# fims9000/SYNT_ISIC

Measured on AMD Instinct MI355X. Metric: images/sec at 3x64x64 T=1000 (DDPM reverse-diffusion sampling), higher is better.
Workload: dtype f32

## Files before the change

synt_isic_amd/csrc/api.cpp:

```cpp
#include <cstring>

#include "common.h"

namespace sisic {

static thread_local char g_err[1024] = "";

void set_error(const char* fmt, ...) {
    va_list ap;
    va_start(ap, fmt);
    vsnprintf(g_err, sizeof(g_err), fmt, ap);
    va_end(ap);
}

static hipEvent_t take_event(sisic_ctx* ctx) {
    if (!ctx->event_pool.empty()) {
        hipEvent_t e = ctx->event_pool.back();
        ctx->event_pool.pop_back();
        return e;
    }
    hipEvent_t e = nullptr;
    if (hipEventCreate(&e) != hipSuccess) return nullptr;
    return e;
}
// ... 52 lines not shown
    *out = nullptr;
    int n = 0;
    SISIC_HIP(hipGetDeviceCount(&n));
    SISIC_REQUIRE(device_id >= 0 && device_id < n, "sisic_create: device %d of %d", device_id, n);
    SISIC_HIP(hipSetDevice(device_id));
    hipDeviceProp_t prop;
    SISIC_HIP(hipGetDeviceProperties(&prop, device_id));
    SISIC_REQUIRE(std::strncmp(prop.gcnArchName, "gfx950", 6) == 0,
                  "sisic_create: device %d is %s; this library is built for gfx950 (MI355X) only", device_id,
                  prop.gcnArchName);
    auto* ctx = new sisic_ctx();
    ctx->device = device_id;
    ctx->num_cus = prop.multiProcessorCount;
    *out = ctx;
    return SISIC_OK;
}

int sisic_destroy(sisic_ctx* ctx) {
    if (!ctx) return SISIC_OK;
    (void)profile_collect(ctx);
    for (auto e : ctx->event_pool) (void)hipEventDestroy(e);
    for (auto& kv : ctx->splitk)
        if (kv.second.p) (void)hipFree(kv.second.p);
    delete ctx;
    return SISIC_OK;
}

int64_t sisic_conv_packed_numel(int Cout, int Cin, int ksize) {
    if (Cout <= 0 || Cin <= 0 || (ksize != 1 && ksize != 3 && ksize != 7)) return -1;
    return conv_packed_floats(Cout, Cin, ksize);
}

int sisic_conv_pack_weights(sisic_ctx* ctx, const float* w, int Cout, int Cin, int ksize, float* packed, void* stream) {
    SISIC_REQUIRE(ctx && w && packed && Cout > 0 && Cin > 0, "conv_pack_weights: bad arguments");
    return launch_conv_pack(ctx, w, Cout, Cin, ksize, packed, static_cast<hipStream_t>(stream));
}

int64_t sisic_conv_s2_numel(int Cout, int Cin) {
    if (Cout <= 0 || Cin <= 0) return -1;
    return conv_s2_packed_floats(Cout, Cin);
}

int sisic_conv_s2_pack(sisic_ctx* ctx, const float* w, int Cout, int Cin, float* out, void* stream) {
    SISIC_REQUIRE(ctx && w && out && Cout > 0 && Cin > 0, "conv_s2_pack: bad arguments");
    return launch_conv_s2_pack(ctx, w, Cout, Cin, out, static_cast<hipStream_t>(stream));
}
// ... 119 lines not shown
```

synt_isic_amd/csrc/common.h:

```cpp
#pragma once

#include <hip/hip_runtime.h>

#include <atomic>
#include <cstdarg>
#include <cstdint>
#include <cstdio>
#include <string>
#include <map>
#include <mutex>
#include <vector>

#include "../../include/sisic.h"

namespace sisic {

void set_error(const char* fmt, ...);

#define SISIC_HIP(call)                                                                   \
    do {                                                                                  \
        hipError_t _e = (call);                                                           \
        if (_e != hipSuccess) {                                                           \
            ::sisic::set_error("%s failed: %s (%s:%d)", #call, hipGetErrorString(_e),     \
                               __FILE__, __LINE__);                                       \
// ... 20 lines not shown
struct ProfileSlot {
    double ms = 0, bytes = 0, flops = 0, flops_exec = 0;
    int64_t launches = 0;
};

struct PendingEvent {
    hipEvent_t start, stop;
    int kind;
    int kind2;
};

}

struct sisic_ctx {
    int device = 0;
    int num_cus = 0;
    bool profiling = false;
    sisic::ProfileSlot prof[sisic::PK_COUNT];
    std::vector<sisic::PendingEvent> pending;
    std::vector<hipEvent_t> event_pool;
    struct SplitK { float* p = nullptr; size_t floats = 0; };
    std::map<hipStream_t, SplitK> splitk;
    std::mutex splitk_mutex;
    std::atomic<uint64_t> scratch_generation{0};
};

namespace sisic {

struct ProfileScope {
    sisic_ctx* ctx;
    hipStream_t stream;
    PendingEvent ev{};
    bool active = false;
    ProfileScope(sisic_ctx* c, hipStream_t s, int kind, double bytes, double flops, double flops_exec = -1.0, int kind2 = -1);
    ~ProfileScope();
};

int profile_collect(sisic_ctx* ctx);

inline int ensure_dynamic_lds(sisic_ctx* ctx, const void* kern, int bytes, std::atomic<uint64_t>& done) {
    const uint64_t bit = uint64_t(1) << (ctx->device & 63);
    if (done.load(std::memory_order_acquire) & bit) return SISIC_OK;
    SISIC_HIP(hipFuncSetAttribute(kern, hipFuncAttributeMaxDynamicSharedMemorySize, bytes));
    done.fetch_or(bit, std::memory_order_release);
    return SISIC_OK;
}
// ... 100 lines not shown
```

synt_isic_amd/csrc/conv_winograd.hip:

```cpp
#include <type_traits>

#include "common.h"
#include "gn_merge.h"
#include "pack_device.h"

#ifndef WINO_TIMING
#define WINO_TIMING 0
#endif
#define WINO_STAMP_SLOTS 10
#if WINO_TIMING
#define WINO_STAMP(slot)                                                                                   \
    do {                                                                                                   \
        unsigned long long t_;                                                                             \
        asm volatile("s_memtime %0\n\ts_waitcnt lgkmcnt(0)" : "=s"(t_)::"memory");                         \
        if (tid == 0) reinterpret_cast<unsigned long long*>(p.stats)[(size_t)blockIdx.x * WINO_STAMP_SLOTS + (slot)] = t_; \
    } while (0)
#else
#define WINO_STAMP(slot) do { } while (0)
#endif
#ifndef WINO_ABLATE
#define WINO_ABLATE 0
#endif

namespace sisic {
// ... 12 lines not shown
    int cout_pad;
    const float* bias;
    int Cout;
    const float* gn_scale;
    const float* gn_shift;
    int gn_silu;
    const float* chan_bias;
    int chan_bias_stride;
    const float* residual;
    int relu;
    float* out;
    float* stats;
    float* part;
    int ksplit;
    int groups_x, groups_y, groups_b, n_co_tiles, nwg, nchunks;
    int stagger;
    const float* fin_gamma;
    const float* fin_beta;
    float* fin_scale;
    float* fin_shift;
    float* fin_mean_rstd;
    int fin_groups;
    float fin_eps;
};

constexpr int W_CIC = 8;
constexpr int W_TILES = 64;
constexpr int W_CO = 64;
constexpr int W_SLAB = W_CIC * 16 * 64;

typedef const __attribute__((address_space(1))) char* gcptr_t;
typedef const __attribute__((address_space(1))) float* gfptr_t;
typedef float v4f_t __attribute__((ext_vector_type(4)));
typedef float v2f_t __attribute__((ext_vector_type(2)));
typedef const __attribute__((address_space(1))) v4f_t* gf4ptr_t;
typedef const __attribute__((address_space(1))) v2f_t* gf2ptr_t;
typedef __attribute__((address_space(1))) float* gfwptr_t;
typedef __attribute__((address_space(1))) v2f_t* gf2wptr_t;
__device__ __forceinline__ gcptr_t uniform_ptr(const void* ptr) {
    const unsigned long long v = reinterpret_cast<unsigned long long>(ptr);
    const unsigned lo = __builtin_amdgcn_readfirstlane((unsigned)v);
    const unsigned hi = __builtin_amdgcn_readfirstlane((unsigned)(v >> 32));
    return (gcptr_t)(((unsigned long long)hi << 32) | lo);
}

__device__ __forceinline__ float wsilu(float v) { return v * __builtin_amdgcn_rcpf(1.0f + __expf(-v)); }
// ... 964 lines not shown
```

synt_isic_amd/csrc/conv_winograd_bf3.inc:

```
template <int PRO>
struct Bf3Geom {
    static constexpr int CO_T = 64, NW = 16, THREADS = 1024;
    static constexpr int TY = 8, TX = 8, TILES = 64;
    static constexpr int HH = 18, HWD = 18, HROW = 20, HPL = 10;
    static constexpr int HPI = HH * HWD;
    static constexpr int HB1 = 2 * HH * HROW;
    static constexpr int CPS = 2 * HB1;
    static constexpr int H_FLOATS = (W_CIC / 2) * CPS;
    static constexpr int TPC = THREADS / W_CIC;
    static constexpr int EPT = (HPI + TPC - 1) / TPC;
    static constexpr int RCO = 16, ROUNDS = CO_T / RCO;
    static constexpr int M_ROUND = 16 * RCO * TILES;
    static constexpr int EPI_FLOATS = 2 * M_ROUND;
    static constexpr int GN_MAX_CH = 2048;
    static constexpr int UA_WAVE = 768;
    static constexpr int UA_BUF = NW * UA_WAVE;
    static constexpr int UA_OFF = H_FLOATS + 2 * GN_MAX_CH;
    static constexpr int LOOP_FLOATS = UA_OFF + 2 * UA_BUF;
    static constexpr int EPI_OFF = H_FLOATS;
    static constexpr int HOFF_OFF = (LOOP_FLOATS > EPI_OFF + EPI_FLOATS ? LOOP_FLOATS : EPI_OFF + EPI_FLOATS);
    static constexpr int FIN_OFF = HOFF_OFF + 2 * THREADS;
    static constexpr size_t LDS_BYTES = sizeof(float) * (size_t)(FIN_OFF + 2 * CO_T);
    static_assert(LDS_BYTES <= 160 * 1024, "bf16x3 Winograd: LDS");
};
// ... 6 lines not shown
#endif
#ifndef BF3Q_VAR
#define BF3Q_VAR 0
#endif
#ifndef BF3_VAR
#define BF3_VAR 0
#endif
#define BF3_STAMPS 16
#if WINO_TIMING
#define BF3_STAMP(slot)                                                                                    \
    do {                                                                                                   \
        unsigned long long t_;                                                                             \
        asm volatile("s_memtime %0\n\ts_waitcnt lgkmcnt(0)" : "=s"(t_)::"memory");                         \
        if (lane == 0) reinterpret_cast<unsigned long long*>(p.stats)[((size_t)BF3_STAMP_ITEM * 16 + wave_u) * BF3_STAMPS + (slot)] = t_; \
    } while (0)
#else
#define BF3_STAMP(slot) do { } while (0)
#endif
typedef short bf3_bf16x8 __attribute__((ext_vector_type(8)));
typedef unsigned bf3_u4 __attribute__((ext_vector_type(4)));
typedef float bf3_f2 __attribute__((ext_vector_type(2)));
typedef unsigned bf3_u2 __attribute__((ext_vector_type(2)));

template <int PRO, bool UPS = false>
__global__ void __launch_bounds__(1024, 4) conv_winograd_bf3_kernel(const WinoParams p) {
    using G = Bf3Geom<PRO>;
    extern __shared__ __attribute__((aligned(16))) float smem[];
    float* const H_lds = smem;
    float* const GN_lds = smem + G::H_FLOATS;
    float* const M_base = smem + G::EPI_OFF;

    int L = blockIdx.x;
    int co_t, gx, gy, b0, oy0, ox0, co0;
    auto decode = [&](const int l) {
        const int nwg = p.nwg;
        const int xcd = l & 7, slot = l >> 3, q = nwg >> 3, r = nwg & 7;
        const int work = (xcd < r ? xcd * (q + 1) : r * (q + 1) + (xcd - r) * q) + slot;
        co_t = work % p.n_co_tiles;
        int grp = work / p.n_co_tiles;
        gx = grp % p.groups_x;
        grp /= p.groups_x;
        gy = grp % p.groups_y;
        b0 = grp / p.groups_y;
        oy0 = gy * 2 * G::TY; ox0 = gx * 2 * G::TX;
        co0 = co_t * G::CO_T;
    };
    decode(L);
    const int n = p.nchunks;
    const int per_img = p.n_co_tiles * p.groups_x * p.groups_y;
    const int img_step = ((p.nwg & 7) == 0 && (int)(gridDim.x >> 3) % per_img == 0) ? (int)(gridDim.x >> 3) / per_img : 0;

    const int tid = threadIdx.x;
    const int lane = tid & 63, wave = tid >> 6;
    const int half = lane >> 5, l31 = lane & 31;
    const int wave_u = __builtin_amdgcn_readfirstlane(wave);
    const int HWin = p.Hin * p.Win, Cin = p.c0 + p.c1;
    auto fresh_lane = [] {
        int l;
        asm volatile("v_mbcnt_lo_u32_b32 %0, -1, 0\n\tv_mbcnt_hi_u32_b32 %0, -1, %0" : "=v"(l));
        return l;
    };
    float* const UA_lds = smem + G::UA_OFF + wave_u * G::UA_WAVE;
    const unsigned ua_lds_addr = __builtin_amdgcn_readfirstlane((unsigned)(size_t)(__attribute__((address_space(3))) float*)UA_lds);

    __amdgpu_buffer_rsrc_t rs0, rs1;
    const __amdgpu_buffer_rsrc_t rsu = __builtin_amdgcn_make_buffer_rsrc(const_cast<float*>(p.uw), 0, -1, 0x00020000);

    const int sci = wave_u >> 1;
    const int sl = tid & 127;
    unsigned goff[G::EPT];
    int hoff[G::EPT];
    auto plan = [&](auto full_tag) {
        constexpr bool FULL = decltype(full_tag)::value;
// ... 7 lines not shown
            const int y = oy0 - 1 + yy, x = ox0 - 1 + xx;
            const bool v = in && y >= 0 && y < p.Hc && x >= 0 && x < p.Wc;
            const int slot = yy * G::HROW + (xx & 1) * G::HPL + (xx >> 1);
            goff[i] = v ? 4u * (unsigned)((y >> (UPS ? 1 : 0)) * p.Win + (x >> (UPS ? 1 : 0))) : 0u;
            if constexpr (FULL) {
                hoff[i] = 2 * (v ? slot : (G::HPL - 1) + G::HPL * (sl_i & 1));
                if (in && !v) {
                    float* z = H_lds + (sci >> 1) * G::CPS + 2 * slot + (sci & 1);
                    z[0] = 0.0f;
                    z[G::HB1] = 0.0f;
                }
            }
        }
        if constexpr (FULL) {
            static_assert(G::EPT == 3, "three store offsets in two dwords");
            *reinterpret_cast<bf3_u2*>(smem + G::HOFF_OFF + 2 * ((wave_u >> 1) * G::TPC + sl_i)) =
                bf3_u2{(unsigned)hoff[0] | ((unsigned)hoff[1] << 16), (unsigned)hoff[2]};
        }
    };
    auto set_sources = [&] {
        rs0 = __builtin_amdgcn_make_buffer_rsrc(const_cast<float*>(p.in0 + (size_t)b0 * p.c0 * HWin), 0, -1, 0x00020000);
        rs1 = __builtin_amdgcn_make_buffer_rsrc(const_cast<float*>(p.in1 ? p.in1 + (size_t)b0 * p.c1 * HWin : p.in0), 0, -1, 0x00020000);
    };
    set_sources();
    plan(std::false_type{});

    const int pos = wave_u, pi = pos >> 2, pj = pos & 3;
    const bool live = !(UPS && (pi == 2 || pj == 2));
    const int ra = (pi == 0) ? 0 : (pi == 2 ? 2 : 1), rb = (pi == 2) ? 1 : (pi == 3 ? 3 : 2);
    const int ca = (pj == 0) ? 0 : (pj == 2 ? 2 : 1), cb = (pj == 2) ? 1 : (pj == 3 ? 3 : 2);
    const float sr = (pi == 1) ? 1.0f : -1.0f, sc = (pj == 1) ? 1.0f : -1.0f;
    const int col_a = (ca & 1) * G::HPL + (ca >> 1), col_b = (cb & 1) * G::HPL + (cb >> 1);
    const float *p_ac, *p_ae, *p_bc, *p_be;
    unsigned u_lane;
    auto lane_addresses = [&] {
        const int ln = fresh_lane();
        const int hf = ln >> 5, t31 = ln & 31, ty = t31 >> 3, tx = t31 & 7;
        const int xf_lane = (2 * hf) * G::CPS + 2 * ((2 * ty) * G::HROW + tx);
        p_ac = H_lds + xf_lane + 2 * (ra * G::HROW + col_a);
        p_ae = H_lds + xf_lane + 2 * (ra * G::HROW + col_b);
        p_bc = H_lds + xf_lane + 2 * (rb * G::HROW + col_a);
        p_be = H_lds + xf_lane + 2 * (rb * G::HROW + col_b);
        u_lane = 16u * (unsigned)ln;
    };
    lane_addresses();

    const int n_co32 = p.cout_pad >> 5;
// ... 115 lines not shown
                acc[x][nb] = __builtin_amdgcn_mfma_f32_32x32x16_bf16(__builtin_bit_cast(bf3_bf16x8, ua[x]), __builtin_bit_cast(bf3_bf16x8, b_mh), acc[x][nb], 0, 0, 0);
                if constexpr ((BF3_VAR & 4096) == 0)
                    acc[x][nb] = __builtin_amdgcn_mfma_f32_32x32x16_bf16(__builtin_bit_cast(bf3_bf16x8, a_hl), __builtin_bit_cast(bf3_bf16x8, b_lh), acc[x][nb], 0, 0, 0);
                if constexpr ((BF3_VAR & 512) != 0) {
                    if constexpr (INIT) {
                        const f32x16 zero = {0.0f, 0.0f, 0.0f, 0.0f, 0.0f, 0.0f, 0.0f, 0.0f, 0.0f, 0.0f, 0.0f, 0.0f, 0.0f, 0.0f, 0.0f, 0.0f};
                        acc[x][1] = __builtin_amdgcn_mfma_f32_32x32x16_bf16(__builtin_bit_cast(bf3_bf16x8, ua[x]), __builtin_bit_cast(bf3_bf16x8, b_hm), zero, 0, 0, 0);
                    } else {
                        acc[x][1] = __builtin_amdgcn_mfma_f32_32x32x16_bf16(__builtin_bit_cast(bf3_bf16x8, ua[x]), __builtin_bit_cast(bf3_bf16x8, b_hm), acc[x][1], 0, 0, 0);
                    }
                    acc[x][1] = __builtin_amdgcn_mfma_f32_32x32x16_bf16(__builtin_bit_cast(bf3_bf16x8, ua[x]), __builtin_bit_cast(bf3_bf16x8, b_mh), acc[x][1], 0, 0, 0);
                    acc[x][1] = __builtin_amdgcn_mfma_f32_32x32x16_bf16(__builtin_bit_cast(bf3_bf16x8, a_hl), __builtin_bit_cast(bf3_bf16x8, b_lh), acc[x][1], 0, 0, 0);
                }
            }
            if constexpr ((BF3_VAR & 256) != 0) __builtin_amdgcn_s_setprio(0);
        }
        __builtin_amdgcn_sched_barrier(0);
    };

    const int cor = wave_u;
    float gn_pre0 = 0.0f, gn_pre1 = 0.0f;
    auto prefetch_gn = [&] {
        if constexpr (PRO != 0) {
            const int ci = b0 * Cin + min(wave_u * 64 + fresh_lane(), Cin - 1);
            gn_pre0 = p.gn_scale[ci];
            gn_pre1 = p.gn_shift[ci];
        }
    };
    auto pin_requests = [&] {
#pragma unroll
        for (int i = 0; i < G::EPT; ++i) asm volatile("" : "+v"(hs[0].v[i]));
#pragma unroll
        for (int i = 0; i < G::EPT; ++i) asm volatile("" : "+v"(hs[1].v[i]));
        if constexpr (PRO != 0) asm volatile("" : "+v"(gn_pre0), "+v"(gn_pre1));
    };
    load_halo(0, hs[0]);
    if (live) fetch_u(0, 0);
    if (n > 1) load_halo(1, hs[1]);
    prefetch_gn();
    pin_requests();
    bool first = true;
    bool new_tile = true;
  for (;;) {
#define BF3_STAMP_ITEM L
    BF3_STAMP(0);
    if constexpr (UPS) {
#pragma unroll
        for (int x = 0; x < 2; ++x)
#pragma unroll
            for (int nb = 0; nb < 2; ++nb)
#pragma unroll
                for (int r = 0; r < 16; ++r) acc[x][nb][r] = 0.0f;
    }
    if (new_tile) plan(std::true_type{});
    {
        const bf3_u2 h = *reinterpret_cast<const bf3_u2*>(smem + G::HOFF_OFF + 2 * (wave_u * 64 + fresh_lane()));
        hoff[0] = (int)(h.x & 0xffffu); hoff[1] = (int)(h.x >> 16); hoff[2] = (int)h.y;
    }
    lane_addresses();
    const float tile_cnt = (float)(min(2 * G::TY, p.Hc - oy0) * min(2 * G::TX, p.Wc - ox0));
    const float inv_cnt = 1.0f / tile_cnt;

    if constexpr (PRO != 0) {
        const int c0t = wave_u * 64 + fresh_lane();
        if (c0t < n * W_CIC) {
            const bool cv = c0t < Cin;
            *reinterpret_cast<bf3_f2*>(GN_lds + 2 * c0t) = bf3_f2{cv ? gn_pre0 : 0.0f, cv ? gn_pre1 : 0.0f};
        }
        for (int c = c0t + G::THREADS; c < n * W_CIC; c += G::THREADS) {
            const bool cv = c < Cin;
            const int ci = b0 * Cin + min(c, Cin - 1);
            const float gsc = p.gn_scale[ci], gsh = p.gn_shift[ci];
            *reinterpret_cast<bf3_f2*>(GN_lds + 2 * c) = bf3_f2{cv ? gsc : 0.0f, cv ? gsh : 0.0f};
        }
    }
    if (!first && live) fetch_u(0, 0);
    first = false;
    if constexpr (PRO != 0) __syncthreads();
    stage_halo(0, 0, hs[0]);
    if (n > 2) load_halo(2, hs[0]);
    __syncthreads();
    BF3_STAMP(1);
    {
        auto body = [&](const int c, auto par_tag, auto steady_tag, auto init_tag) {
            constexpr int PAR = decltype(par_tag)::value;
            constexpr bool STEADY = decltype(steady_tag)::value;
            if (c == 2 + PAR) BF3_STAMP(2 + 4 * PAR);
            if constexpr (BF3_PRIO != 0) __builtin_amdgcn_s_setprio(3);
            if (live) {
                if constexpr ((BF3_VAR & 1) == 0) {
                    read_u(BF3_ONE_UA ? 0 : PAR, std::integral_constant<int, STEADY ? 3 : 0>{}, c == 0 && n > 2);
                    if constexpr (BF3_ONE_UA != 0) {
                        if (STEADY || c + 1 < n) {
                            asm volatile("s_waitcnt lgkmcnt(0)" ::: "memory");
                            fetch_u(c + 1, 0);
                        }
                    }
                }
            }
            if (live) compute_half(PAR, std::integral_constant<int, 0>{}, init_tag);
            if (STEADY || c + 1 < n) {
                if constexpr ((BF3_VAR & 4) == 0) stage_halo(c + 1, PAR ^ 1, hs[PAR ^ 1]);
                if constexpr ((BF3_VAR & 1) == 0 && BF3_ONE_UA == 0)
                    if (live) fetch_u(c + 1, PAR ^ 1);
// ... 13 lines not shown
        c = 1;
        for (; c + 4 < n; c += 2) {
            body(c, std::integral_constant<int, 1>{}, std::true_type{}, std::false_type{});
            body(c + 1, std::integral_constant<int, 0>{}, std::true_type{}, std::false_type{});
        }
        if (c < n) body(c, std::integral_constant<int, 1>{}, std::false_type{}, std::false_type{});
        if (c + 1 < n) body(c + 1, std::integral_constant<int, 0>{}, std::false_type{}, std::false_type{});
        if (c + 2 < n) body(c + 2, std::integral_constant<int, 1>{}, std::false_type{}, std::false_type{});
        if (c + 3 < n) body(c + 3, std::integral_constant<int, 0>{}, std::false_type{}, std::false_type{});
    }

    BF3_STAMP(10);
    if constexpr ((BF3_VAR & 16) != 0) {
        float t = 0.0f;
#pragma unroll
        for (int x = 0; x < 2; ++x)
#pragma unroll
            for (int nb = 0; nb < 2; ++nb)
#pragma unroll
                for (int r = 0; r < 16; ++r) t += acc[x][nb][r];
        if (t == 123.456f) p.out[tid] = t;
        return;
    }
    float eadd_v = 0.0f;
    {
        const int ln = fresh_lane();
        const int coc = min(co0 + (ln & 3) * G::RCO + cor, p.Cout - 1);
        const float* src = ln < 4 ? (p.bias ? p.bias + coc : nullptr)
                                  : (ln < 8 && p.chan_bias ? p.chan_bias + (size_t)b0 * p.chan_bias_stride + coc : nullptr);
        if (src) eadd_v = *src;
    }
    const int HWo = p.Hc * p.Wc;
    const int et = fresh_lane(), e_half = et >> 5, e_l31 = et & 31;
    const int ety = et >> 3, etx = et & 7;
    const int eoy = oy0 + 2 * ety, eox = ox0 + 2 * etx;
    const bool even_w = (p.Wc & 1) == 0;
    const bool has_res = p.residual != nullptr;
    unsigned ld_off[2][2], st_off[2][2];
    bool pin[2][2];
#pragma unroll
    for (int i = 0; i < 2; ++i)
#pragma unroll
        for (int j = 0; j < 2; ++j) {
            pin[i][j] = eoy + i < p.Hc && eox + j < p.Wc;
            ld_off[i][j] = 4u * (unsigned)(min(eoy + i, p.Hc - 1) * p.Wc + min(eox + j, p.Wc - (even_w ? 2 - j : 1)));
            st_off[i][j] = pin[i][j] ? ld_off[i][j] : 0x80000000u;
        }
    const __amdgpu_buffer_rsrc_t rso = __builtin_amdgcn_make_buffer_rsrc(p.out + (size_t)b0 * p.Cout * HWo, 0, 4 * p.Cout * HWo, 0x00020000);
    const __amdgpu_buffer_rsrc_t rsr = __builtin_amdgcn_make_buffer_rsrc(
        const_cast<float*>(has_res ? p.residual + (size_t)b0 * p.Cout * HWo : p.out), 0, 4 * p.Cout * HWo, 0x00020000);

    bf3_f2 eres[G::ROUNDS][2];
#pragma unroll
    for (int q = 0; q < G::ROUNDS; ++q) {
        const int coc = min(co0 + q * G::RCO + cor, p.Cout - 1);
        const unsigned soff = 4u * (unsigned)(coc * HWo);
#pragma unroll
        for (int i = 0; i < 2; ++i) eres[q][i] = bf3_f2{0.0f, 0.0f};
        if (has_res) {
            if (even_w) {
#pragma unroll
                for (int i = 0; i < 2; ++i)
                    eres[q][i] = __builtin_bit_cast(bf3_f2, __builtin_amdgcn_raw_buffer_load_b64(rsr, ld_off[i][0], soff, 0));
            } else {
#pragma unroll
                for (int i = 0; i < 2; ++i) {
                    eres[q][i].x = __builtin_bit_cast(float, __builtin_amdgcn_raw_buffer_load_b32(rsr, ld_off[i][0], soff, 0));
                    eres[q][i].y = __builtin_bit_cast(float, __builtin_amdgcn_raw_buffer_load_b32(rsr, ld_off[i][1], soff, 0));
                }
            }
        }
    }
    float eadd[G::ROUNDS];
#pragma unroll
    for (int q = 0; q < G::ROUNDS; ++q)
        eadd[q] = (0.0f + __uint_as_float(__builtin_amdgcn_readlane(__float_as_uint(eadd_v), q))) +
                  __uint_as_float(__builtin_amdgcn_readlane(__float_as_uint(eadd_v), 4 + q));
    const int co0_c = co0, b0_c = b0, slot_c = gy * p.groups_x + gx;
    const int L_next = L + (int)gridDim.x;
    const bool more = L_next < p.nwg;
    if (more) {
        const int gx_c = gx, gy_c = gy;
        if (img_step) b0 += img_step;
        else decode(L_next);
        set_sources();
        new_tile = gx != gx_c || gy != gy_c;
        if (new_tile) plan(std::false_type{});
        load_halo(0, hs[0]);
        if (n > 1) load_halo(1, hs[1]);
        prefetch_gn();
    }
#pragma unroll
    for (int q = 0; q < G::ROUNDS; ++q) {
        float* const M_lds = M_base + (q & 1) * G::M_ROUND;
        if (q == 0) BF3_STAMP(11);
        {
            const int rbase = 8 * (q & 1);
#pragma unroll
            for (int nb = 0; nb < 2; ++nb)
#pragma unroll
                for (int rr = 0; rr < 8; ++rr) {
                    const int r = rbase + rr;
                    const int row16 = (r & 3) + 8 * ((r >> 2) & 1) + 4 * e_half;
                    M_lds[(pos * G::RCO + row16) * G::TILES + 32 * nb + e_l31] = acc[q >> 1][nb][r];
                }
        }
        if (q == 0) BF3_STAMP(12);
        __syncthreads();
        if (q == 0) BF3_STAMP(13);
        float mm[4][4];
#pragma unroll
        for (int xi = 0; xi < 16; ++xi) mm[xi >> 2][xi & 3] = M_lds[(xi * G::RCO + cor) * G::TILES + et];
        float sT[2][4];
// ... 6 lines not shown
#pragma unroll
        for (int i = 0; i < 2; ++i) {
            vv[i][0] = sT[i][0] + sT[i][1] + sT[i][2] + eadd[q] + eres[q][i].x;
            vv[i][1] = sT[i][1] - sT[i][2] - sT[i][3] + eadd[q] + eres[q][i].y;
            if (p.relu) { vv[i][0] = fmaxf(vv[i][0], 0.0f); vv[i][1] = fmaxf(vv[i][1], 0.0f); }
        }
        const int co = co0_c + q * G::RCO + cor;
        const bool ok = co < p.Cout;
        const unsigned soff = 4u * (unsigned)(min(co, p.Cout - 1) * HWo);
        if (q == G::ROUNDS - 1) pin_requests();
        if (even_w) {
#pragma unroll
            for (int i = 0; i < 2; ++i)
                __builtin_amdgcn_raw_buffer_store_b64(bf3_u2{__float_as_uint(vv[i][0]), __float_as_uint(vv[i][1])}, rso, ok ? st_off[i][0] : 0x80000000u, soff, 0);
        } else {
#pragma unroll
            for (int i = 0; i < 2; ++i) {
                __builtin_amdgcn_raw_buffer_store_b32(__float_as_uint(vv[i][0]), rso, ok ? st_off[i][0] : 0x80000000u, soff, 0);
                __builtin_amdgcn_raw_buffer_store_b32(__float_as_uint(vv[i][1]), rso, ok ? st_off[i][1] : 0x80000000u, soff, 0);
            }
        }
        if (q == 0) BF3_STAMP(14);
        if (!WINO_TIMING && (p.stats || (!UPS && p.fin_gamma))) {
            const float K = __shfl(vv[0][0], 0);
            float s1 = 0.0f, s2 = 0.0f;
#pragma unroll
            for (int i = 0; i < 2; ++i) {
                const float d0 = pin[i][0] ? vv[i][0] - K : 0.0f, d1 = pin[i][1] ? vv[i][1] - K : 0.0f;
                s1 += d0 + d1;
                s2 = fmaf(d0, d0, fmaf(d1, d1, s2));
            }
            s1 = wave64_sum(s1);
            s2 = wave64_sum(s2);
            if (ok && et == 0) {
                const float p_sum = fmaf(tile_cnt, K, s1), p_m2 = fmaxf(s2 - s1 * s1 * inv_cnt, 0.0f);
                if (p.stats) {
                    const int slots = p.groups_x * p.groups_y;
                    float4* dst = reinterpret_cast<float4*>(p.stats) + ((size_t)b0_c * p.Cout + co) * slots + slot_c;
                    *dst = make_float4(tile_cnt, p_sum, p_m2, 0.0f);
                }
                if (!UPS && p.fin_gamma) *reinterpret_cast<bf3_f2*>(smem + G::FIN_OFF + 2 * (q * G::RCO + cor)) = bf3_f2{p_sum, p_m2};
            }
        }
    }
#if WINO_TIMING
    if (!more) asm volatile("s_waitcnt vmcnt(0)" ::: "memory");
#endif
    BF3_STAMP(15);
#undef BF3_STAMP_ITEM
    if (!UPS && p.fin_gamma) {
        __syncthreads();
        const int c = tid;
        if (c < G::CO_T) {
            const bf3_f2* ps = reinterpret_cast<const bf3_f2*>(smem + G::FIN_OFF) + 8 * (c >> 3);
            double pn[8], s1v[8], m2v[8];
#pragma unroll
            for (int i = 0; i < 8; ++i) { pn[i] = (double)tile_cnt + (double)0.0f; s1v[i] = (double)ps[i].x + (double)0.0f; m2v[i] = (double)ps[i].y + (double)0.0f; }
            auto tree = [](const double (&v)[8]) { return ((v[0] + v[1]) + (v[2] + v[3])) + ((v[4] + v[5]) + (v[6] + v[7])); };
            const double nn = tree(pn), sum1 = tree(s1v), sum2 = tree(m2v);
            const double mean = sum1 / nn;
            double bt[8];
#pragma unroll
            for (int i = 0; i < 8; ++i) bt[i] = 0.0 + gn_between_term(tile_cnt, ps[i].x, mean);
            const double between = tree(bt);
            float meanf, rstd;
            gn_mean_rstd(nn, sum1, sum2, between, p.fin_eps, meanf, rstd, mean);
            const int co = co0_c + c;
            float sc, sh;
            gn_affine(p.fin_gamma[co], p.fin_beta[co], meanf, rstd, sc, sh);
            p.fin_scale[(size_t)b0_c * p.Cout + co] = sc;
            p.fin_shift[(size_t)b0_c * p.Cout + co] = sh;
            if (p.fin_mean_rstd && (c & 7) == 0) {
                p.fin_mean_rstd[2 * ((size_t)b0_c * p.fin_groups + (co >> 3))] = meanf;
                p.fin_mean_rstd[2 * ((size_t)b0_c * p.fin_groups + (co >> 3)) + 1] = rstd;
            }
        }
    }
    if (!more) break;
    L = L_next;
    __syncthreads();
  }
}

#define BF3_STAMP_ITEM blockIdx.x
struct Bf3QGeom {
    static constexpr int CO_T = 64, NW = 16, THREADS = 1024, TILES = 64, IMGS = 4;
    static constexpr int HH = 10, HWD = 10, HROW = 12, HPL = 6;
    static constexpr int HPI = HH * HWD;
    static constexpr int IMG = 2 * HH * HROW + 8;
    static constexpr int HB1 = IMGS * IMG;
    static constexpr int CPS = 2 * HB1;
    static constexpr int H_FLOATS = (W_CIC / 2) * CPS;
    static constexpr int GN_MAX_CH = 512;
    static constexpr int UA_WAVE = 768, UA_BUF = NW * UA_WAVE;
// ... 293 lines not shown
            const unsigned soff = 4u * (unsigned)(co * HWo);
            if (even_w) {
#pragma unroll
                for (int i = 0; i < 2; ++i)
                    __builtin_amdgcn_raw_buffer_store_b64(bf3_u2{__float_as_uint(vv[i][0]), __float_as_uint(vv[i][1])}, rso, st_off[i][0], soff, 0);
            } else {
#pragma unroll
                for (int i = 0; i < 2; ++i) {
                    __builtin_amdgcn_raw_buffer_store_b32(__float_as_uint(vv[i][0]), rso, st_off[i][0], soff, 0);
                    __builtin_amdgcn_raw_buffer_store_b32(__float_as_uint(vv[i][1]), rso, st_off[i][1], soff, 0);
                }
            }
        }
    }
}

__global__ void winograd_pack_bf3_kernel(const float* __restrict__ u_first, int cin_pad, int cout_pad, int cout_pad128,
                                         unsigned* __restrict__ out) {
    const size_t total = (size_t)(cin_pad / 8) * 16 * (cout_pad128 / 64) * 768;
    for (size_t i = (size_t)blockIdx.x * blockDim.x + threadIdx.x; i < total; i += (size_t)gridDim.x * blockDim.x)
        winograd_pack_bf3_elem(i, u_first, cout_pad, cout_pad128, out);
}

template <int PRO, bool UPS>
static int launch_bf3(sisic_ctx* ctx, WinoParams& p, hipStream_t s) {
    using G = Bf3Geom<PRO>;
    p.groups_x = cdiv(p.Wc, 2 * G::TX);
    p.groups_y = cdiv(p.Hc, 2 * G::TY);
    p.groups_b = p.B;
    p.n_co_tiles = cdiv(p.Cout, G::CO_T);
    p.nchunks = cdiv(p.c0 + p.c1, W_CIC);
    p.ksplit = 1;
    const int64_t nwg = (int64_t)p.groups_x * p.groups_y * p.groups_b * p.n_co_tiles;
    SISIC_REQUIRE(nwg > 0 && nwg < (int64_t(1) << 31), "conv2d(winograd bf16x3): grid too large");
    SISIC_REQUIRE((double)round_up(p.c0 + p.c1, 16) * 32.0 * p.cout_pad * 4.0 < 4294967296.0, "conv2d(winograd bf16x3): filter tensor too large for 32-bit offsets");
    SISIC_REQUIRE((double)p.Cout * p.Hc * p.Wc * 4.0 < 2147483648.0, "conv2d(winograd bf16x3): one image of the output is too large for 31-bit offsets");
    SISIC_REQUIRE(p.nchunks * W_CIC <= G::GN_MAX_CH, "conv2d(winograd bf16x3): more than %d input channels", G::GN_MAX_CH);
    p.nwg = (int)nwg;
    auto kern = conv_winograd_bf3_kernel<PRO, UPS>;
    static std::atomic<uint64_t> lds_opt_in{0};
    SISIC_TRY(ensure_dynamic_lds(ctx, reinterpret_cast<const void*>(kern), (int)G::LDS_BYTES, lds_opt_in));
    static const bool persistent = [] { const char* e = std::getenv("SISIC_BF3_PERSISTENT"); return !e || std::atoi(e) != 0; }();
    const int cus = ctx->num_cus > 0 ? ctx->num_cus & ~7 : 256;
    const int grid = (persistent && p.nwg > cus && cus >= 8) ? cus : p.nwg;
    hipLaunchKernelGGL(kern, dim3(grid), dim3(G::THREADS), G::LDS_BYTES, s, p);
    SISIC_HIP(hipGetLastError());
    return SISIC_OK;
}

template <int PRO>
static int launch_bf3q(sisic_ctx* ctx, WinoParams& p, hipStream_t s) {
    using G = Bf3QGeom;
    p.n_co_tiles = cdiv(p.Cout, G::CO_T);
    p.nchunks = cdiv(p.c0 + p.c1, W_CIC);
    const int64_t nwg = (int64_t)cdiv(p.B, G::IMGS) * p.n_co_tiles * p.ksplit;
    SISIC_REQUIRE(nwg > 0 && nwg < (int64_t(1) << 31), "conv2d(winograd bf16x3, 8x8): grid too large");
    SISIC_REQUIRE(p.nchunks % p.ksplit == 0 && p.nchunks * W_CIC <= G::GN_MAX_CH,
                  "conv2d(winograd bf16x3, 8x8): needs a multiple of %d and at most %d input channels", p.ksplit * W_CIC, G::GN_MAX_CH);
    SISIC_REQUIRE(4.0 * G::IMGS * std::max(p.c0, p.c1) * p.Hin * p.Win < 4294967296.0 && 4.0 * G::IMGS * p.Cout * p.Hc * p.Wc < 2147483648.0,
                  "conv2d(winograd bf16x3, 8x8): tensor too large for 32-bit offsets");
    p.nwg = (int)nwg;
    auto kern = conv_winograd_bf3q_kernel<PRO>;
    static std::atomic<uint64_t> lds_opt_in{0};
    SISIC_TRY(ensure_dynamic_lds(ctx, reinterpret_cast<const void*>(kern), (int)G::LDS_BYTES, lds_opt_in));
    hipLaunchKernelGGL(kern, dim3(p.nwg), dim3(G::THREADS), G::LDS_BYTES, s, p);
    SISIC_HIP(hipGetLastError());
    return SISIC_OK;
}
// ... 20 lines not shown
```

Measured before the change: 12.53.

## Precompute per-work-item descriptor table for persistent bf16x3 Winograd conv

Adds a cached device-side table of 64-byte work-item records (offsets, tile flags, counts, stats/fin offsets) built once per shape by a small kernel. The persistent bf16x3 Winograd kernel loads each record with one scalar fetch instead of decoding indices and computing offsets with integer division, and it loads bias and embedding values through scalar loads. The intent is to cut scalar/integer overhead and latency in the epilogue and at work-item transitions. In exchange it adds host-side table management (mutex, events, capture checks), a second kernel variant, and extra device memory.

```diff
diff --git a/synt_isic_amd/csrc/api.cpp b/synt_isic_amd/csrc/api.cpp
--- a/synt_isic_amd/csrc/api.cpp
+++ b/synt_isic_amd/csrc/api.cpp
@@ -98,6 +98,10 @@
     for (auto e : ctx->event_pool) (void)hipEventDestroy(e);
     for (auto& kv : ctx->splitk)
         if (kv.second.p) (void)hipFree(kv.second.p);
+    for (auto& it : ctx->bf3_items) {
+        if (it.fill_done) (void)hipEventDestroy(it.fill_done);
+        if (it.tab) (void)hipFree(it.tab);
+    }
     delete ctx;
     return SISIC_OK;
 }
diff --git a/synt_isic_amd/csrc/common.h b/synt_isic_amd/csrc/common.h
--- a/synt_isic_amd/csrc/common.h
+++ b/synt_isic_amd/csrc/common.h
@@ -66,6 +66,9 @@
     struct SplitK { float* p = nullptr; size_t floats = 0; };
     std::map<hipStream_t, SplitK> splitk;
     std::mutex splitk_mutex;
+    struct Bf3Items { int key[9]; unsigned* tab = nullptr; hipStream_t fill_stream = nullptr; hipEvent_t fill_done = nullptr; };
+    std::vector<Bf3Items> bf3_items;
+    std::mutex bf3_items_mutex;
     std::atomic<uint64_t> scratch_generation{0};
 };
 
diff --git a/synt_isic_amd/csrc/conv_winograd.hip b/synt_isic_amd/csrc/conv_winograd.hip
--- a/synt_isic_amd/csrc/conv_winograd.hip
+++ b/synt_isic_amd/csrc/conv_winograd.hip
@@ -58,6 +58,8 @@
     float* fin_mean_rstd;
     int fin_groups;
     float fin_eps;
+    int grid;
+    const unsigned* items;
 };
 
 constexpr int W_CIC = 8;
diff --git a/synt_isic_amd/csrc/conv_winograd_bf3.inc b/synt_isic_amd/csrc/conv_winograd_bf3.inc
--- a/synt_isic_amd/csrc/conv_winograd_bf3.inc
+++ b/synt_isic_amd/csrc/conv_winograd_bf3.inc
@@ -52,7 +52,78 @@
 typedef float bf3_f2 __attribute__((ext_vector_type(2)));
 typedef unsigned bf3_u2 __attribute__((ext_vector_type(2)));
 
-template <int PRO, bool UPS = false>
+struct Bf3Item {
+    unsigned b0, co0, oy0, ox0;
+    unsigned slot;
+    unsigned in0_off, in1_off;
+    unsigned out_off;
+    unsigned gn_off;
+    unsigned cb_off;
+    unsigned stats_off;
+    unsigned fin_off;
+    unsigned flags;
+    unsigned tile_cnt, inv_cnt;
+    unsigned tile_off;
+};
+static_assert(sizeof(Bf3Item) == 64, "one s_load_dwordx16 per record");
+enum : unsigned {
+    BF3_IT_WHOLE = 1,
+    BF3_IT_EVEN_W = 2,
+    BF3_IT_NEW_TILE = 4,
+    BF3_IT_LAST = 8,
+};
+typedef unsigned bf3_u16 __attribute__((ext_vector_type(16)));
+__device__ __forceinline__ bf3_u16 bf3_item_fetch(const unsigned* tab, int L) {
+    asm volatile("" : "+s"(L));
+    return *(reinterpret_cast<const __attribute__((address_space(4))) bf3_u16*>((size_t)tab) + L);
+}
+#define BF3_IT(rec, field) ((rec)[offsetof(Bf3Item, field) / 4])
+
+__device__ __forceinline__ void bf3_decode(const WinoParams& p, int l, int& co_t, int& gx, int& gy, int& b0) {
+    const int nwg = p.nwg;
+    const int xcd = l & 7, slot = l >> 3, q = nwg >> 3, r = nwg & 7;
+    const int work = (xcd < r ? xcd * (q + 1) : r * (q + 1) + (xcd - r) * q) + slot;
+    co_t = work % p.n_co_tiles;
+    int grp = work / p.n_co_tiles;
+    gx = grp % p.groups_x;
+    grp /= p.groups_x;
+    gy = grp % p.groups_y;
+    b0 = grp / p.groups_y;
+}
+
+__global__ void bf3_item_table_kernel(const WinoParams p, unsigned* __restrict__ tab) {
+    const int L = blockIdx.x * blockDim.x + threadIdx.x;
+    if (L >= p.nwg) return;
+    int co_t, gx, gy, b0;
+    bf3_decode(p, L, co_t, gx, gy, b0);
+    const int oy0 = gy * 16, ox0 = gx * 16, co0 = co_t * 64;
+    const unsigned HWin = (unsigned)(p.Hin * p.Win), HWo = (unsigned)(p.Hc * p.Wc), slots = (unsigned)(p.groups_x * p.groups_y);
+    Bf3Item it;
+    it.b0 = (unsigned)b0; it.co0 = (unsigned)co0; it.oy0 = (unsigned)oy0; it.ox0 = (unsigned)ox0;
+    it.slot = (unsigned)(gy * p.groups_x + gx);
+    it.in0_off = (unsigned)b0 * (unsigned)p.c0 * HWin;
+    it.in1_off = (unsigned)b0 * (unsigned)p.c1 * HWin;
+    it.out_off = (unsigned)b0 * (unsigned)p.Cout * HWo;
+    it.gn_off = (unsigned)b0 * (unsigned)(p.c0 + p.c1);
+    it.cb_off = (unsigned)b0 * (unsigned)p.chan_bias_stride;
+    it.stats_off = ((unsigned)b0 * (unsigned)p.Cout + (unsigned)co0) * slots + it.slot;
+    it.fin_off = (unsigned)b0 * (unsigned)p.Cout + (unsigned)co0;
+    bool new_tile = true;
+    if (L >= p.grid) {
+        int co_p, gx_p, gy_p, b_p;
+        bf3_decode(p, L - p.grid, co_p, gx_p, gy_p, b_p);
+        new_tile = gx != gx_p || gy != gy_p;
+    }
+    it.flags = ((oy0 + 16 <= p.Hc && ox0 + 16 <= p.Wc) ? BF3_IT_WHOLE : 0u) | ((p.Wc & 1) == 0 ? BF3_IT_EVEN_W : 0u) |
+               (new_tile ? BF3_IT_NEW_TILE : 0u) | (L + p.grid >= p.nwg ? BF3_IT_LAST : 0u);
+    const float tile_cnt = (float)(min(16, p.Hc - oy0) * min(16, p.Wc - ox0));
+    it.tile_cnt = __float_as_uint(tile_cnt);
+    it.inv_cnt = __float_as_uint(1.0f / tile_cnt);
+    it.tile_off = 4u * (unsigned)(oy0 * p.Wc + ox0);
+    reinterpret_cast<Bf3Item*>(tab)[L] = it;
+}
+
+template <int PRO, bool UPS = false, bool TAB = false>
 __global__ void __launch_bounds__(1024, 4) conv_winograd_bf3_kernel(const WinoParams p) {
     using G = Bf3Geom<PRO>;
     extern __shared__ __attribute__((aligned(16))) float smem[];
@@ -75,10 +146,13 @@
         oy0 = gy * 2 * G::TY; ox0 = gx * 2 * G::TX;
         co0 = co_t * G::CO_T;
     };
-    decode(L);
+    if constexpr (!TAB) decode(L);
     const int n = p.nchunks;
-    const int per_img = p.n_co_tiles * p.groups_x * p.groups_y;
-    const int img_step = ((p.nwg & 7) == 0 && (int)(gridDim.x >> 3) % per_img == 0) ? (int)(gridDim.x >> 3) / per_img : 0;
+    int img_step = 0;
+    if constexpr (!TAB) {
+        const int per_img = p.n_co_tiles * p.groups_x * p.groups_y;
+        img_step = ((p.nwg & 7) == 0 && (int)(gridDim.x >> 3) % per_img == 0) ? (int)(gridDim.x >> 3) / per_img : 0;
+    }
 
     const int tid = threadIdx.x;
     const int lane = tid & 63, wave = tid >> 6;
@@ -132,7 +206,20 @@
         rs0 = __builtin_amdgcn_make_buffer_rsrc(const_cast<float*>(p.in0 + (size_t)b0 * p.c0 * HWin), 0, -1, 0x00020000);
         rs1 = __builtin_amdgcn_make_buffer_rsrc(const_cast<float*>(p.in1 ? p.in1 + (size_t)b0 * p.c1 * HWin : p.in0), 0, -1, 0x00020000);
     };
-    set_sources();
+    auto set_sources_item = [&](const bf3_u16& it) {
+        rs0 = __builtin_amdgcn_make_buffer_rsrc(const_cast<float*>(p.in0 + (size_t)BF3_IT(it, in0_off)), 0, -1, 0x00020000);
+        rs1 = __builtin_amdgcn_make_buffer_rsrc(const_cast<float*>(p.in1 ? p.in1 + (size_t)BF3_IT(it, in1_off) : p.in0), 0, -1, 0x00020000);
+    };
+    int gn_base = 0;
+    if constexpr (TAB) {
+        const bf3_u16 it = bf3_item_fetch(p.items, L);
+        b0 = (int)BF3_IT(it, b0); co0 = (int)BF3_IT(it, co0); co_t = co0 >> 6; oy0 = (int)BF3_IT(it, oy0); ox0 = (int)BF3_IT(it, ox0);
+        gx = gy = 0;
+        set_sources_item(it);
+        gn_base = (int)BF3_IT(it, gn_off);
+    } else {
+        set_sources();
+    }
     plan(std::false_type{});
 
     const int pos = wave_u, pi = pos >> 2, pj = pos & 3;
@@ -294,7 +381,7 @@
     float gn_pre0 = 0.0f, gn_pre1 = 0.0f;
     auto prefetch_gn = [&] {
         if constexpr (PRO != 0) {
-            const int ci = b0 * Cin + min(wave_u * 64 + fresh_lane(), Cin - 1);
+            const int ci = (TAB ? gn_base : b0 * Cin) + min(wave_u * 64 + fresh_lane(), Cin - 1);
             gn_pre0 = p.gn_scale[ci];
             gn_pre1 = p.gn_shift[ci];
         }
@@ -330,8 +417,13 @@
         hoff[0] = (int)(h.x & 0xffffu); hoff[1] = (int)(h.x >> 16); hoff[2] = (int)h.y;
     }
     lane_addresses();
-    const float tile_cnt = (float)(min(2 * G::TY, p.Hc - oy0) * min(2 * G::TX, p.Wc - ox0));
-    const float inv_cnt = 1.0f / tile_cnt;
+    float tile_cnt = 0.0f, inv_cnt = 0.0f;
+    if constexpr (!TAB) {
+        tile_cnt = (float)(min(2 * G::TY, p.Hc - oy0) * min(2 * G::TX, p.Wc - ox0));
+        inv_cnt = 1.0f / tile_cnt;
+    }
+    unsigned it_warm = 0;
+    if constexpr (TAB) it_warm = bf3_item_fetch(p.items, min(L + p.grid, p.nwg - 1))[0];
 
     if constexpr (PRO != 0) {
         const int c0t = wave_u * 64 + fresh_lane();
@@ -341,7 +433,7 @@
         }
         for (int c = c0t + G::THREADS; c < n * W_CIC; c += G::THREADS) {
             const bool cv = c < Cin;
-            const int ci = b0 * Cin + min(c, Cin - 1);
+            const int ci = (TAB ? gn_base : b0 * Cin) + min(c, Cin - 1);
             const float gsc = p.gn_scale[ci], gsh = p.gn_shift[ci];
             *reinterpret_cast<bf3_f2*>(GN_lds + 2 * c) = bf3_f2{cv ? gsc : 0.0f, cv ? gsh : 0.0f};
         }
@@ -352,6 +444,7 @@
     stage_halo(0, 0, hs[0]);
     if (n > 2) load_halo(2, hs[0]);
     __syncthreads();
+    if constexpr (TAB) asm volatile("" :: "s"(it_warm));
     BF3_STAMP(1);
     {
         auto body = [&](const int c, auto par_tag, auto steady_tag, auto init_tag) {
@@ -411,73 +504,166 @@
         if (t == 123.456f) p.out[tid] = t;
         return;
     }
-    float eadd_v = 0.0f;
-    {
-        const int ln = fresh_lane();
-        const int coc = min(co0 + (ln & 3) * G::RCO + cor, p.Cout - 1);
-        const float* src = ln < 4 ? (p.bias ? p.bias + coc : nullptr)
-                                  : (ln < 8 && p.chan_bias ? p.chan_bias + (size_t)b0 * p.chan_bias_stride + coc : nullptr);
-        if (src) eadd_v = *src;
-    }
     const int HWo = p.Hc * p.Wc;
     const int et = fresh_lane(), e_half = et >> 5, e_l31 = et & 31;
     const int ety = et >> 3, etx = et & 7;
-    const int eoy = oy0 + 2 * ety, eox = ox0 + 2 * etx;
-    const bool even_w = (p.Wc & 1) == 0;
     const bool has_res = p.residual != nullptr;
+    bool even_w;
     unsigned ld_off[2][2], st_off[2][2];
     bool pin[2][2];
-#pragma unroll
-    for (int i = 0; i < 2; ++i)
-#pragma unroll
-        for (int j = 0; j < 2; ++j) {
-            pin[i][j] = eoy + i < p.Hc && eox + j < p.Wc;
-            ld_off[i][j] = 4u * (unsigned)(min(eoy + i, p.Hc - 1) * p.Wc + min(eox + j, p.Wc - (even_w ? 2 - j : 1)));
-            st_off[i][j] = pin[i][j] ? ld_off[i][j] : 0x80000000u;
-        }
-    const __amdgpu_buffer_rsrc_t rso = __builtin_amdgcn_make_buffer_rsrc(p.out + (size_t)b0 * p.Cout * HWo, 0, 4 * p.Cout * HWo, 0x00020000);
-    const __amdgpu_buffer_rsrc_t rsr = __builtin_amdgcn_make_buffer_rsrc(
-        const_cast<float*>(has_res ? p.residual + (size_t)b0 * p.Cout * HWo : p.out), 0, 4 * p.Cout * HWo, 0x00020000);
-
+    __amdgpu_buffer_rsrc_t rso;
     bf3_f2 eres[G::ROUNDS][2];
-#pragma unroll
-    for (int q = 0; q < G::ROUNDS; ++q) {
-        const int coc = min(co0 + q * G::RCO + cor, p.Cout - 1);
-        const unsigned soff = 4u * (unsigned)(coc * HWo);
-#pragma unroll
-        for (int i = 0; i < 2; ++i) eres[q][i] = bf3_f2{0.0f, 0.0f};
+    float eadd[G::ROUNDS];
+    int co0_c, b0_c, slot_c, L_next;
+    bool more;
+    unsigned stats_base = 0, fin_base = 0;
+    if constexpr (TAB) {
+        const bf3_u16 it = bf3_item_fetch(p.items, L);
+        const bf3_u16 nx = bf3_item_fetch(p.items, min(L + p.grid, p.nwg - 1));
+        const unsigned flags = BF3_IT(it, flags);
+        co0_c = (int)BF3_IT(it, co0); b0_c = (int)BF3_IT(it, b0); slot_c = (int)BF3_IT(it, slot);
+        stats_base = BF3_IT(it, stats_off); fin_base = BF3_IT(it, fin_off);
+        tile_cnt = __uint_as_float(BF3_IT(it, tile_cnt)); inv_cnt = __uint_as_float(BF3_IT(it, inv_cnt));
+        even_w = (flags & BF3_IT_EVEN_W) != 0;
+        unsigned coc4[G::ROUNDS];
+        unsigned ebias[G::ROUNDS], eemb[G::ROUNDS];
+#pragma unroll
+        for (int q = 0; q < G::ROUNDS; ++q) {
+            coc4[q] = (unsigned)min(co0_c + q * G::RCO + cor, p.Cout - 1);
+            ebias[q] = 0u; eemb[q] = 0u;
+        }
+        typedef const __attribute__((address_space(4))) unsigned* cbits_ptr;
+        if (p.bias) {
+#pragma unroll
+            for (int q = 0; q < G::ROUNDS; ++q) ebias[q] = reinterpret_cast<cbits_ptr>((size_t)p.bias)[coc4[q]];
+        }
+        if (p.chan_bias) {
+            cbits_ptr cb = reinterpret_cast<cbits_ptr>((size_t)p.chan_bias) + BF3_IT(it, cb_off);
+#pragma unroll
+            for (int q = 0; q < G::ROUNDS; ++q) eemb[q] = cb[coc4[q]];
+        }
+        if ((flags & (BF3_IT_WHOLE | BF3_IT_EVEN_W)) == (BF3_IT_WHOLE | BF3_IT_EVEN_W)) {
+            const unsigned o = BF3_IT(it, tile_off) + (unsigned)ety * (8u * (unsigned)p.Wc) + 8u * (unsigned)etx;
+#pragma unroll
+            for (int i = 0; i < 2; ++i)
+#pragma unroll
+                for (int j = 0; j < 2; ++j) {
+                    pin[i][j] = true;
+                    ld_off[i][j] = st_off[i][j] = o + (unsigned)i * (4u * (unsigned)p.Wc) + 4u * (unsigned)j;
+                }
+        } else {
+            const int eoy = (int)BF3_IT(it, oy0) + 2 * ety, eox = (int)BF3_IT(it, ox0) + 2 * etx;
+#pragma unroll
+            for (int i = 0; i < 2; ++i)
+#pragma unroll
+                for (int j = 0; j < 2; ++j) {
+                    pin[i][j] = eoy + i < p.Hc && eox + j < p.Wc;
+                    ld_off[i][j] = 4u * (unsigned)(min(eoy + i, p.Hc - 1) * p.Wc + min(eox + j, p.Wc - (even_w ? 2 - j : 1)));
+                    st_off[i][j] = pin[i][j] ? ld_off[i][j] : 0x80000000u;
+                }
+        }
+        rso = __builtin_amdgcn_make_buffer_rsrc(p.out + (size_t)BF3_IT(it, out_off), 0, 4 * p.Cout * HWo, 0x00020000);
+        const __amdgpu_buffer_rsrc_t rsr = __builtin_amdgcn_make_buffer_rsrc(
+            const_cast<float*>(has_res ? p.residual + (size_t)BF3_IT(it, out_off) : p.out), 0, 4 * p.Cout * HWo, 0x00020000);
+#pragma unroll
+        for (int q = 0; q < G::ROUNDS; ++q)
+#pragma unroll
+            for (int i = 0; i < 2; ++i) eres[q][i] = bf3_f2{0.0f, 0.0f};
         if (has_res) {
             if (even_w) {
 #pragma unroll
-                for (int i = 0; i < 2; ++i)
-                    eres[q][i] = __builtin_bit_cast(bf3_f2, __builtin_amdgcn_raw_buffer_load_b64(rsr, ld_off[i][0], soff, 0));
+                for (int q = 0; q < G::ROUNDS; ++q)
+#pragma unroll
+                    for (int i = 0; i < 2; ++i)
+                        eres[q][i] = __builtin_bit_cast(bf3_f2, __builtin_amdgcn_raw_buffer_load_b64(rsr, ld_off[i][0], 4u * (coc4[q] * (unsigned)HWo), 0));
             } else {
 #pragma unroll
-                for (int i = 0; i < 2; ++i) {
-                    eres[q][i].x = __builtin_bit_cast(float, __builtin_amdgcn_raw_buffer_load_b32(rsr, ld_off[i][0], soff, 0));
-                    eres[q][i].y = __builtin_bit_cast(float, __builtin_amdgcn_raw_buffer_load_b32(rsr, ld_off[i][1], soff, 0));
+                for (int q = 0; q < G::ROUNDS; ++q)
+#pragma unroll
+                    for (int i = 0; i < 2; ++i) {
+                        eres[q][i].x = __builtin_bit_cast(float, __builtin_amdgcn_raw_buffer_load_b32(rsr, ld_off[i][0], 4u * (coc4[q] * (unsigned)HWo), 0));
+                        eres[q][i].y = __builtin_bit_cast(float, __builtin_amdgcn_raw_buffer_load_b32(rsr, ld_off[i][1], 4u * (coc4[q] * (unsigned)HWo), 0));
+                    }
+            }
+        }
+        L_next = L + p.grid;
+        more = (flags & BF3_IT_LAST) == 0;
+        if (more) {
+            b0 = (int)BF3_IT(nx, b0); co0 = (int)BF3_IT(nx, co0); co_t = co0 >> 6; oy0 = (int)BF3_IT(nx, oy0); ox0 = (int)BF3_IT(nx, ox0);
+            gn_base = (int)BF3_IT(nx, gn_off);
+            set_sources_item(nx);
+            new_tile = (BF3_IT(nx, flags) & BF3_IT_NEW_TILE) != 0;
+            if (new_tile) plan(std::false_type{});
+            load_halo(0, hs[0]);
+            if (n > 1) load_halo(1, hs[1]);
+            prefetch_gn();
+        }
+#pragma unroll
+        for (int q = 0; q < G::ROUNDS; ++q) {
+            asm volatile("" : "+s"(ebias[q]), "+s"(eemb[q]));
+            eadd[q] = (0.0f + __uint_as_float(ebias[q])) + __uint_as_float(eemb[q]);
+        }
+    } else {
+        float eadd_v = 0.0f;
+        {
+            const int ln = fresh_lane();
+            const int coc = min(co0 + (ln & 3) * G::RCO + cor, p.Cout - 1);
+            const float* src = ln < 4 ? (p.bias ? p.bias + coc : nullptr)
+                                      : (ln < 8 && p.chan_bias ? p.chan_bias + (size_t)b0 * p.chan_bias_stride + coc : nullptr);
+            if (src) eadd_v = *src;
+        }
+        const int eoy = oy0 + 2 * ety, eox = ox0 + 2 * etx;
+        even_w = (p.Wc & 1) == 0;
+#pragma unroll
+        for (int i = 0; i < 2; ++i)
+#pragma unroll
+            for (int j = 0; j < 2; ++j) {
+                pin[i][j] = eoy + i < p.Hc && eox + j < p.Wc;
+                ld_off[i][j] = 4u * (unsigned)(min(eoy + i, p.Hc - 1) * p.Wc + min(eox + j, p.Wc - (even_w ? 2 - j : 1)));
+                st_off[i][j] = pin[i][j] ? ld_off[i][j] : 0x80000000u;
+            }
+        rso = __builtin_amdgcn_make_buffer_rsrc(p.out + (size_t)b0 * p.Cout * HWo, 0, 4 * p.Cout * HWo, 0x00020000);
+        const __amdgpu_buffer_rsrc_t rsr = __builtin_amdgcn_make_buffer_rsrc(
+            const_cast<float*>(has_res ? p.residual + (size_t)b0 * p.Cout * HWo : p.out), 0, 4 * p.Cout * HWo, 0x00020000);
+
+#pragma unroll
+        for (int q = 0; q < G::ROUNDS; ++q) {
+            const int coc = min(co0 + q * G::RCO + cor, p.Cout - 1);
+            const unsigned soff = 4u * (unsigned)(coc * HWo);
+#pragma unroll
+            for (int i = 0; i < 2; ++i) eres[q][i] = bf3_f2{0.0f, 0.0f};
+            if (has_res) {
+                if (even_w) {
+#pragma unroll
+                    for (int i = 0; i < 2; ++i)
+                        eres[q][i] = __builtin_bit_cast(bf3_f2, __builtin_amdgcn_raw_buffer_load_b64(rsr, ld_off[i][0], soff, 0));
+                } else {
+#pragma unroll
+                    for (int i = 0; i < 2; ++i) {
+                        eres[q][i].x = __builtin_bit_cast(float, __builtin_amdgcn_raw_buffer_load_b32(rsr, ld_off[i][0], soff, 0));
+                        eres[q][i].y = __builtin_bit_cast(float, __builtin_amdgcn_raw_buffer_load_b32(rsr, ld_off[i][1], soff, 0));
+                    }
                 }
             }
         }
-    }
-    float eadd[G::ROUNDS];
-#pragma unroll
-    for (int q = 0; q < G::ROUNDS; ++q)
-        eadd[q] = (0.0f + __uint_as_float(__builtin_amdgcn_readlane(__float_as_uint(eadd_v), q))) +
-                  __uint_as_float(__builtin_amdgcn_readlane(__float_as_uint(eadd_v), 4 + q));
-    const int co0_c = co0, b0_c = b0, slot_c = gy * p.groups_x + gx;
-    const int L_next = L + (int)gridDim.x;
-    const bool more = L_next < p.nwg;
-    if (more) {
-        const int gx_c = gx, gy_c = gy;
-        if (img_step) b0 += img_step;
-        else decode(L_next);
-        set_sources();
-        new_tile = gx != gx_c || gy != gy_c;
-        if (new_tile) plan(std::false_type{});
-        load_halo(0, hs[0]);
-        if (n > 1) load_halo(1, hs[1]);
-        prefetch_gn();
+#pragma unroll
+        for (int q = 0; q < G::ROUNDS; ++q)
+            eadd[q] = (0.0f + __uint_as_float(__builtin_amdgcn_readlane(__float_as_uint(eadd_v), q))) +
+                      __uint_as_float(__builtin_amdgcn_readlane(__float_as_uint(eadd_v), 4 + q));
+        co0_c = co0; b0_c = b0; slot_c = gy * p.groups_x + gx;
+        L_next = L + (int)gridDim.x;
+        more = L_next < p.nwg;
+        if (more) {
+            const int gx_c = gx, gy_c = gy;
+            if (img_step) b0 += img_step;
+            else decode(L_next);
+            set_sources();
+            new_tile = gx != gx_c || gy != gy_c;
+            if (new_tile) plan(std::false_type{});
+            load_halo(0, hs[0]);
+            if (n > 1) load_halo(1, hs[1]);
+            prefetch_gn();
+        }
     }
 #pragma unroll
     for (int q = 0; q < G::ROUNDS; ++q) {
@@ -530,7 +716,7 @@
         }
         if (q == 0) BF3_STAMP(14);
         if (!WINO_TIMING && (p.stats || (!UPS && p.fin_gamma))) {
-            const float K = __shfl(vv[0][0], 0);
+            const float K = TAB ? __uint_as_float(__builtin_amdgcn_readlane(__float_as_uint(vv[0][0]), 0)) : __shfl(vv[0][0], 0);
             float s1 = 0.0f, s2 = 0.0f;
 #pragma unroll
             for (int i = 0; i < 2; ++i) {
@@ -544,7 +730,8 @@
                 const float p_sum = fmaf(tile_cnt, K, s1), p_m2 = fmaxf(s2 - s1 * s1 * inv_cnt, 0.0f);
                 if (p.stats) {
                     const int slots = p.groups_x * p.groups_y;
-                    float4* dst = reinterpret_cast<float4*>(p.stats) + ((size_t)b0_c * p.Cout + co) * slots + slot_c;
+                    float4* dst = TAB ? reinterpret_cast<float4*>(p.stats) + ((size_t)stats_base + (size_t)((q * G::RCO + cor) * slots))
+                                      : reinterpret_cast<float4*>(p.stats) + ((size_t)b0_c * p.Cout + co) * slots + slot_c;
                     *dst = make_float4(tile_cnt, p_sum, p_m2, 0.0f);
                 }
                 if (!UPS && p.fin_gamma) *reinterpret_cast<bf3_f2*>(smem + G::FIN_OFF + 2 * (q * G::RCO + cor)) = bf3_f2{p_sum, p_m2};
@@ -558,7 +745,7 @@
 #undef BF3_STAMP_ITEM
     if (!UPS && p.fin_gamma) {
         __syncthreads();
-        const int c = tid;
+        const int c = TAB ? wave_u * 64 + fresh_lane() : tid;
         if (c < G::CO_T) {
             const bf3_f2* ps = reinterpret_cast<const bf3_f2*>(smem + G::FIN_OFF) + 8 * (c >> 3);
             double pn[8], s1v[8], m2v[8];
@@ -576,8 +763,9 @@
             const int co = co0_c + c;
             float sc, sh;
             gn_affine(p.fin_gamma[co], p.fin_beta[co], meanf, rstd, sc, sh);
-            p.fin_scale[(size_t)b0_c * p.Cout + co] = sc;
-            p.fin_shift[(size_t)b0_c * p.Cout + co] = sh;
+            const size_t fi = TAB ? (size_t)fin_base + (size_t)c : (size_t)b0_c * p.Cout + co;
+            p.fin_scale[fi] = sc;
+            p.fin_shift[fi] = sh;
             if (p.fin_mean_rstd && (c & 7) == 0) {
                 p.fin_mean_rstd[2 * ((size_t)b0_c * p.fin_groups + (co >> 3))] = meanf;
                 p.fin_mean_rstd[2 * ((size_t)b0_c * p.fin_groups + (co >> 3)) + 1] = rstd;
@@ -917,6 +1105,50 @@
         winograd_pack_bf3_elem(i, u_first, cout_pad, cout_pad128, out);
 }
 
+static int bf3_item_table(sisic_ctx* ctx, WinoParams& p, hipStream_t s) {
+    constexpr size_t MAX_TABLES = 48, MAX_BYTES = size_t(8) << 20;
+    const char* e = std::getenv("SISIC_BF3_ITEM_TABLE");
+    if (e && std::atoi(e) == 0) return SISIC_OK;
+    const double HWin = (double)p.Hin * p.Win, HWo = (double)p.Hc * p.Wc, lim = 4294967296.0;
+    const double slots = (double)p.groups_x * p.groups_y;
+    if ((double)p.B * std::max(p.c0, p.c1) * HWin >= lim || (double)p.B * p.Cout * HWo >= lim || (double)p.B * (p.c0 + p.c1) >= lim ||
+        (double)p.B * std::max(p.chan_bias_stride, 0) >= lim || (double)p.B * round_up(p.Cout, 64) * slots >= lim || p.chan_bias_stride < 0 ||
+        (size_t)p.nwg * sizeof(Bf3Item) > MAX_BYTES)
+        return SISIC_OK;
+    const int key[9] = {p.B, p.Hin, p.Win, p.ups, p.c0, p.c1, p.Cout, p.grid, p.chan_bias_stride};
+    std::lock_guard<std::mutex> lock(ctx->bf3_items_mutex);
+    hipStreamCaptureStatus cap = hipStreamCaptureStatusNone;
+    SISIC_HIP(hipStreamIsCapturing(s, &cap));
+    for (auto& it : ctx->bf3_items) {
+        if (!std::equal(key, key + 9, it.key)) continue;
+        if (it.fill_done && cap == hipStreamCaptureStatusNone && hipEventQuery(it.fill_done) == hipSuccess) {
+            (void)hipEventDestroy(it.fill_done);
+            it.fill_done = nullptr;
+        }
+        if (!it.fill_done || it.fill_stream == s) p.items = it.tab;
+        return SISIC_OK;
+    }
+    if (ctx->bf3_items.size() >= MAX_TABLES || cap != hipStreamCaptureStatusNone) return SISIC_OK;
+    sisic_ctx::Bf3Items ent;
+    std::copy(key, key + 9, ent.key);
+    SISIC_HIP(hipMalloc(reinterpret_cast<void**>(&ent.tab), (size_t)p.nwg * sizeof(Bf3Item)));
+    hipLaunchKernelGGL(bf3_item_table_kernel, dim3(cdiv(p.nwg, 256)), dim3(256), 0, s, p, ent.tab);
+    if (hipGetLastError() != hipSuccess) {
+        (void)hipFree(ent.tab);
+        set_error("conv2d(winograd bf16x3): item table kernel failed to launch");
+        return SISIC_EHIP;
+    }
+    ent.fill_stream = s;
+    if (hipEventCreateWithFlags(&ent.fill_done, hipEventDisableTiming) != hipSuccess || hipEventRecord(ent.fill_done, s) != hipSuccess) {
+        if (ent.fill_done) (void)hipEventDestroy(ent.fill_done);
+        ent.fill_done = nullptr;
+        SISIC_HIP(hipStreamSynchronize(s));
+    }
+    ctx->bf3_items.push_back(ent);
+    p.items = ent.tab;
+    return SISIC_OK;
+}
+
 template <int PRO, bool UPS>
 static int launch_bf3(sisic_ctx* ctx, WinoParams& p, hipStream_t s) {
     using G = Bf3Geom<PRO>;
@@ -932,13 +1164,23 @@
     SISIC_REQUIRE((double)p.Cout * p.Hc * p.Wc * 4.0 < 2147483648.0, "conv2d(winograd bf16x3): one image of the output is too large for 31-bit offsets");
     SISIC_REQUIRE(p.nchunks * W_CIC <= G::GN_MAX_CH, "conv2d(winograd bf16x3): more than %d input channels", G::GN_MAX_CH);
     p.nwg = (int)nwg;
-    auto kern = conv_winograd_bf3_kernel<PRO, UPS>;
-    static std::atomic<uint64_t> lds_opt_in{0};
-    SISIC_TRY(ensure_dynamic_lds(ctx, reinterpret_cast<const void*>(kern), (int)G::LDS_BYTES, lds_opt_in));
     static const bool persistent = [] { const char* e = std::getenv("SISIC_BF3_PERSISTENT"); return !e || std::atoi(e) != 0; }();
     const int cus = ctx->num_cus > 0 ? ctx->num_cus & ~7 : 256;
     const int grid = (persistent && p.nwg > cus && cus >= 8) ? cus : p.nwg;
-    hipLaunchKernelGGL(kern, dim3(grid), dim3(G::THREADS), G::LDS_BYTES, s, p);
+    p.grid = grid;
+    p.items = nullptr;
+    SISIC_TRY(bf3_item_table(ctx, p, s));
+    if (p.items) {
+        auto kern = conv_winograd_bf3_kernel<PRO, UPS, true>;
+        static std::atomic<uint64_t> lds_opt_in{0};
+        SISIC_TRY(ensure_dynamic_lds(ctx, reinterpret_cast<const void*>(kern), (int)G::LDS_BYTES, lds_opt_in));
+        hipLaunchKernelGGL(kern, dim3(grid), dim3(G::THREADS), G::LDS_BYTES, s, p);
+    } else {
+        auto kern = conv_winograd_bf3_kernel<PRO, UPS, false>;
+        static std::atomic<uint64_t> lds_opt_in{0};
+        SISIC_TRY(ensure_dynamic_lds(ctx, reinterpret_cast<const void*>(kern), (int)G::LDS_BYTES, lds_opt_in));
+        hipLaunchKernelGGL(kern, dim3(grid), dim3(G::THREADS), G::LDS_BYTES, s, p);
+    }
     SISIC_HIP(hipGetLastError());
     return SISIC_OK;
 }
```

Measured after the change: 12.69, median of 6. +1.3%, better.
